# slp-rl/aero

Hardware: NVIDIA H100
Metric: audio-seconds/sec forward (higher is better)
Workload: dtype f16 tensor-core operands and activation storage (10-bit mantissa = tf32), fp32 accumulate / norm inputs / cell state

## Files before the change

### aero_b200/cabi.py

```python
from __future__ import annotations

import ctypes as C
import os

_HERE = os.path.dirname(os.path.abspath(__file__))
LIB_PATH = os.path.join(_HERE, "libaero_b200.so")

i32, i64, f32 = C.c_int32, C.c_int64, C.c_float
vp = C.c_void_p


class StftParams(C.Structure):
    _fields_ = [("n_fft", i32), ("hop", i32), ("win", i32), ("n_signals", i32), ("channels", i32),
                ("length", i32), ("frames", i32), ("bins_out", i32),
                ("z_stride_b", i64), ("z_stride_c", i64), ("z_stride_k", i64), ("z_stride_t", i64),
                ("flags", i32), ("reserved", i32)]


class IstftParams(C.Structure):
    _fields_ = [("n_fft", i32), ("hop", i32), ("win", i32), ("n_signals", i32), ("channels", i32),
                ("frames", i32), ("bins_in", i32), ("out_len", i32),
                ("z_stride_b", i64), ("z_stride_c", i64), ("z_stride_k", i64), ("z_stride_t", i64),
                ("flags", i32), ("reserved", i32)]

# ... 47 lines not shown
ACT_NONE, ACT_GELU, ACT_RELU, ACT_LEAKY, ACT_TANH = 0, 1, 2, 3, 4
TG_ROUND_TF32, TG_A_F16, TG_OUT_F16, TG_REVERSE = 1, 2, 4, 8
NA_NONE, NA_GELU, NA_GLU, NA_SNAKE, NA_GLU_SCALE_RES, NA_RELU, NA_LEAKY, NA_TANH = 0, 1, 2, 3, 4, 5, 6, 7
NA_NO_NORM = 16
STFT_ZERO_PAD, STFT_ADJ_SCALE, ISTFT_RAW = 1, 2, 1
GAN_NONE, GAN_LSGAN_REAL, GAN_LSGAN_FAKE, GAN_LSGAN_GEN, GAN_HINGE_REAL, GAN_HINGE_FAKE, GAN_HINGE_GEN = 0, 1, 2, 3, 4, 5, 6
GAN_FWD_BLOCKS = 128

SYMBOLS = {
    "aero_abi_version": (C.c_int, []),
    "aero_last_error": (C.c_char_p, []),
    "aero_device_arch": (C.c_int, []),
    "aero_launch_count": (C.c_uint64, []),
    "aero_stft_fwd": (C.c_int, [vp, vp, vp, vp, C.POINTER(StftParams), vp]),
    "aero_istft_fwd": (C.c_int, [vp, vp, vp, C.POINTER(IstftParams), vp]),
    "aero_tapgemm_fwd": (C.c_int, [vp] * 10 + [C.POINTER(TapGemmParams), vp]),
    "aero_tapgemm_tc_eligible": (C.c_int, [C.POINTER(TapGemmParams)]),
    "aero_sample_norm_fwd": (C.c_int, [vp, vp, vp, vp, i32, i64, i64, i32, vp]),
    "aero_norm_act_fwd": (C.c_int, [vp] * 8 + [C.POINTER(NormActParams), vp]),
    "aero_ftb_lin_out_fwd": (C.c_int, [vp] * 7 + [C.POINTER(FtbLinParams), vp]),
    "aero_ftb_lin_squeeze_fwd": (C.c_int, [vp, vp, vp, vp, i32, C.POINTER(FtbLinParams), vp]),
    "aero_freq_mix_small_fwd": (C.c_int, [vp, vp, vp, vp, i32, i32, i64, i32, vp]),
    "aero_lstm_rec_fwd": (C.c_int, [vp, vp, vp, vp, C.POINTER(LstmParams), vp]),
    "aero_local_attn_fwd": (C.c_int, [vp, vp, C.POINTER(AttnParams), vp]),
    "aero_lsd_fwd": (C.c_int, [vp, vp, vp, i32, i32, i32, i32, vp]),
    "aero_stft_loss_fwd": (C.c_int, [vp, vp, vp, i32, i32, i32, i32, vp]),
    "aero_stft_loss_bwd": (C.c_int, [vp, vp, vp, vp, i32, i32, i32, i32, f32, f32, vp]),
    "aero_tapgemm_wgrad": (C.c_int, [vp, vp, vp, vp, C.POINTER(TapGemmParams), i64, i64, i64, vp]),
    "aero_colsum": (C.c_int, [vp, vp, vp, vp, i32, i32, i64, i64, i64, i64, i32, i64, i64, vp]),
    "aero_add": (C.c_int, [vp, vp, i64, f32, vp]),
    "aero_add_f64": (C.c_int, [vp, vp, i64, vp]),
    "aero_gram": (C.c_int, [vp, vp, vp, vp, i32, i32, i64, i64, i64, i64, vp]),
    "aero_bcast_add": (C.c_int, [vp, vp, i32, i32, i32, i32, vp]),
    "aero_scale_rows": (C.c_int, [vp, vp, vp, i32, i64, i32, vp]),
    "aero_norm_act_train_fwd": (C.c_int, [vp] * 8 + [C.POINTER(NormActParams), vp]),
    "aero_norm_act_train_bwd": (C.c_int, [vp] * 13 + [i32, C.POINTER(NormActParams), vp]),
    "aero_adam_step": (C.c_int, [vp, i32, f32, f32, f32, f32, i32, f32, vp]),
    "aero_pack_kmajor_tf32": (C.c_int, [vp, vp, vp, i32, i32, i32, vp]),
    "aero_split_tf32": (C.c_int, [vp, vp, vp, i64, vp]),
    "aero_tapgemm_wgrad_tc_eligible": (C.c_int, [C.POINTER(TapGemmParams), vp, vp, vp]),
    "aero_gconv1d_fwd": (C.c_int, [vp, vp, vp, vp] + [i32] * 9 + [vp]),
    "aero_gconv1d_dgrad": (C.c_int, [vp, vp, vp] + [i32] * 9 + [vp]),
    "aero_gconv1d_wgrad": (C.c_int, [vp, vp, vp] + [i32] * 9 + [vp]),
    "aero_weight_norm_fwd": (C.c_int, [vp, vp, vp, i32, i32, vp]),
    "aero_weight_norm_bwd": (C.c_int, [vp, vp, vp, vp, vp, i32, i32, vp]),
    "aero_lstm_train_fwd": (C.c_int, [vp] * 7 + [C.POINTER(LstmParams), vp]),
# ... 54 lines not shown
```

### aero_b200/csrc/lstm_tc.cu

```cuda
#include <cuda_fp16.h>
#include <cstdlib>
#include "tc_common.cuh"

#ifdef AERO_TC_TRACE
__device__ long long g_lstm_trace[128 * 8];
#define LSTM_TRACE(slot, step) do { if (blockIdx.x == 0 && blockIdx.y == 0 && (step) < 128) g_lstm_trace[(step) * 8 + (slot)] = clock64(); } while (0)
extern "C" int aero_debug_lstm_trace(long long* host) {
    return cudaMemcpyFromSymbol(host, g_lstm_trace, sizeof(g_lstm_trace)) == cudaSuccess ? 0 : -1;
}
#else
#define LSTM_TRACE(slot, step) do { } while (0)
#endif

namespace aero {

constexpr int kNT = 16;
constexpr int kLdAcc = kNT + 4;

static int lstm_seq_knob() {
    static const int v = [] { const char* e = getenv("AERO_LSTM_SEQ"); return e ? atoi(e) : 0; }();
    return v;
}

struct LstmTcShared {
    uint64_t w_full;
    uint64_t acc_ready;
    uint64_t h_ready;
};

__device__ __forceinline__ float fast_ex2(float x) {
    float y;
    asm("ex2.approx.ftz.f32 %0, %1;" : "=f"(y) : "f"(x));
    return y;
}
__device__ __forceinline__ float fast_rcp(float x) {
    float y;
    asm("rcp.approx.ftz.f32 %0, %1;" : "=f"(y) : "f"(x));
    return y;
}

template <typename T> __device__ __forceinline__ T to_storage(float v);
template <> __device__ __forceinline__ float to_storage<float>(float v) { return v; }
template <> __device__ __forceinline__ __half to_storage<__half>(float v) { return __float2half_rn(v); }

template <int GPT, int NEW, int SEQ, int ROWB, int MINB, typename TO, typename TG>
__global__ void __launch_bounds__(128 + 32 * NEW, MINB)
lstm_tc_kernel(const __grid_constant__ CUtensorMap mapW, const TG* __restrict__ gin, const float* __restrict__ bias_pad,
               TO* __restrict__ hout, const aero_lstm_params p, const int nK) {
    constexpr int NM = 4 / GPT;
    constexpr int CPW = 32 / GPT;
    constexpr int kNS = 4 * SEQ / NEW;
    constexpr int kATile = 128 * ROWB, kBTile = kNT * ROWB, kKC = ROWB / 2;
    extern __shared__ uint8_t smem_raw[];
    uint8_t* smem = reinterpret_cast<uint8_t*>((reinterpret_cast<uintptr_t>(smem_raw) + 1023) & ~(uintptr_t)1023);
    uint8_t* sA = smem;
    uint8_t* sB = smem + NM * nK * kATile;
    float* sAcc = reinterpret_cast<float*>(sB + nK * kBTile);
    LstmTcShared* sh = reinterpret_cast<LstmTcShared*>(sAcc + NM * 128 * kLdAcc);

    const int warp = threadIdx.x >> 5, lane = threadIdx.x & 31;
    const int dir = blockIdx.y;
    const int seq0 = blockIdx.x * SEQ;
    const int n_seq = p.rows * p.n_win;
    const int H = p.H;
    const int ldg = 8 * H;

    if (threadIdx.x == 0) {
        mbar_init(&sh->w_full, 1);
        mbar_init(&sh->acc_ready, 128);
        mbar_init(&sh->h_ready, 32 * NEW);
        asm volatile("fence.mbarrier_init.release.cluster;" ::: "memory");
    }
    for (int i = threadIdx.x; i < nK * kBTile / 4; i += blockDim.x) reinterpret_cast<float*>(sB)[i] = 0.f;
    fence_proxy_async_smem();
    __syncthreads();

    if (warp < 4) {
        if (threadIdx.x == 0) {
            asm volatile("prefetch.tensormap [%0];" ::"l"(&mapW) : "memory");
            mbar_expect_tx(&sh->w_full, (uint32_t)(NM * nK * kATile));
            for (int m = 0; m < NM; ++m)
                for (int kc = 0; kc < nK; ++kc)
                    tma_load_2d(sA + (m * nK + kc) * kATile, &mapW, &sh->w_full, kc * kKC, (dir * NM + m) * 128);
        }
        constexpr int kMaxKC = (ROWB == 128) ? 2 : 4;
        uint64_t da[NM][kMaxKC], db[kMaxKC];
        const uint32_t a0 = smem_u32(sA), b0 = smem_u32(sB);
#pragma unroll
        for (int kc = 0; kc < kMaxKC; ++kc) {
            db[kc] = make_desc_kmajor<ROWB>(b0 + (uint32_t)(kc * kBTile));
#pragma unroll
            for (int m = 0; m < NM; ++m) da[m][kc] = make_desc_kmajor<ROWB>(a0 + (uint32_t)((m * nK + kc) * kATile));
        }
        float* const arow = sAcc + (warp * 16 + (lane >> 2)) * kLdAcc + 2 * (lane & 3);
        mbar_wait(&sh->w_full, 0);
        for (int s = 1; s < p.steps; ++s) {
            mbar_wait(&sh->h_ready, (uint32_t)((s - 1) & 1));
            LSTM_TRACE(0, s);
            float d[NM][2][8];
            wgmma_fence();
#pragma unroll
            for (int m = 0; m < NM; ++m) {
#pragma unroll
                for (int hf = 0; hf < 2; ++hf) {
#pragma unroll
                    for (int kc = 0; kc < kMaxKC; ++kc) {
                        if (kc < nK) {
#pragma unroll
                            for (int k = 0; k < ROWB / 32; ++k)
                                Wgmma<kNT, true, 0>::ss(d[m][hf], da[m][kc] + (uint64_t)(hf * ((64 * ROWB) >> 4) + 2 * k), db[kc] + 2 * k,
                                                        (kc == 0 && k == 0) ? 0u : 1u);
                        }
                    }
                }
            }
            wgmma_commit();
            wgmma_wait<0>();
#pragma unroll
            for (int m = 0; m < NM; ++m)
#pragma unroll
                for (int hf = 0; hf < 2; ++hf)
#pragma unroll
                    for (int j = 0; j < 2; ++j) {
                        float* r = arow + (m * 128 + hf * 64) * kLdAcc + 8 * j;
                        *reinterpret_cast<float2*>(r) = make_float2(d[m][hf][4 * j], d[m][hf][4 * j + 1]);
                        *reinterpret_cast<float2*>(r + 8 * kLdAcc) = make_float2(d[m][hf][4 * j + 2], d[m][hf][4 * j + 3]);
                    }
            mbar_arrive(&sh->acc_ready);
            LSTM_TRACE(1, s);
        }
    } else {
        const int ew = warp - 4;
        const int q = warp & 3;
        const int wp = ew >> 2;
        const int sub = lane / CPW;
        const int cell = q * CPW + (lane % CPW);
        const bool cell_ok = cell < H;
        const int r = q * 32 + lane;
        const int half = p.win_stride / 2;
        const int dpos = dir ? -1 : 1;
        const int pos0 = dir ? p.steps - 1 : 0;

        const int gcol = dir * 4 * H + sub * H + min(cell, H - 1);
        const int gtile = GPT * H;
        constexpr int kMS = kNS / GPT;
        int goff[kNS], g_lo[kNS], g_len[kNS];
        int ooff[kMS], w_lo[kMS], w_len[kMS];
        uint32_t baddr[kMS];
        const int jq = (cell & (kKC - 1)) >> 3;
        const uint32_t bbase = smem_u32(sB) + (uint32_t)((cell / kKC) * kBTile + ((cell & 7) << 1));
#pragma unroll
        for (int i = 0; i < kNS; ++i) {
            const int n = wp * kNS + i;
            const int sq = min(seq0 + n, n_seq - 1);
            const int row = sq / p.n_win, k = sq - row * p.n_win;
            const int f0 = k * p.win_stride;
            goff[i] = (p.in_windowed ? (sq * p.steps + pos0) : (row * p.T + f0 + pos0)) * ldg + gcol;
            const int in_hi = p.in_windowed ? p.steps : max(0, min(p.steps, p.T - f0));
            g_lo[i] = dir ? p.steps - in_hi : 0;
            g_len[i] = in_hi;
        }
#pragma unroll
        for (int ii = 0; ii < kMS; ++ii) {
            const int n = wp * kNS + ii * GPT + sub;
            const int sq = min(seq0 + n, n_seq - 1);
            const bool exists = seq0 + n < n_seq;
            const int row = sq / p.n_win, k = sq - row * p.n_win;
            const int f0 = k * p.win_stride;
            ooff[ii] = (p.out_windowed ? (sq * p.steps + pos0) : (row * p.T + f0 + pos0)) * 2 * H + dir * H + cell;
            int lo = 0, hi = p.steps;
            if (!p.out_windowed) {
                lo = (k == 0) ? 0 : half;
                hi = min((k == p.n_win - 1) ? p.steps : p.steps - half, p.T - f0);
            }
            if (!exists || !cell_ok) hi = lo;
            w_lo[ii] = dir ? p.steps - hi : lo;
            w_len[ii] = max(0, hi - lo);
            baddr[ii] = bbase + (uint32_t)((n >> 3) * (8 * ROWB) + (n & 7) * ROWB + ((jq ^ (ROWB == 128 ? (n & 7) : ((n >> 1) & 3))) << 4));
        }
        const float* bptr = bias_pad + gcol;
        const int gstep = dpos * ldg, ostep = dpos * 2 * H;

        float c_state[kMS];
#pragma unroll
        for (int i = 0; i < kMS; ++i) c_state[i] = 0.f;

        constexpr bool kRegPrefetch = (GPT == 1);
        TG gn[kRegPrefetch ? NM : 1][kRegPrefetch ? kNS : 1];
        const TG* const bptr_g = nullptr;
        (void)bptr_g;
        if (kRegPrefetch) {
#pragma unroll
            for (int i = 0; i < kNS; ++i) {
                const bool real = (unsigned)(0 - g_lo[i]) < (unsigned)g_len[i];
#pragma unroll
                for (int m = 0; m < NM; ++m) gn[kRegPrefetch ? m : 0][kRegPrefetch ? i : 0] = real ? gin[goff[i] + m * gtile] : to_storage<TG>(bptr[m * gtile]);
                goff[i] += gstep;
            }
        }
        for (int s = 0; s < p.steps; ++s) {
            float gi[NM][kNS];
            if (kRegPrefetch) {
#pragma unroll
                for (int i = 0; i < kNS; ++i) {
#pragma unroll
                    for (int m = 0; m < NM; ++m) gi[m][i] = ldf(&gn[kRegPrefetch ? m : 0][kRegPrefetch ? i : 0]);
                }
                if (s + 1 < p.steps) {
#pragma unroll
                    for (int i = 0; i < kNS; ++i) {
                        const bool real = (unsigned)(s + 1 - g_lo[i]) < (unsigned)g_len[i];
#pragma unroll
                        for (int m = 0; m < NM; ++m) gn[kRegPrefetch ? m : 0][kRegPrefetch ? i : 0] = real ? gin[goff[i] + m * gtile] : to_storage<TG>(bptr[m * gtile]);
                        goff[i] += gstep;
                    }
                }
            } else {
#pragma unroll
                for (int i = 0; i < kNS; ++i) {
                    const bool real = (unsigned)(s - g_lo[i]) < (unsigned)g_len[i];
#pragma unroll
                    for (int m = 0; m < NM; ++m) gi[m][i] = real ? ldf(gin + goff[i] + m * gtile) : bptr[m * gtile];
                    goff[i] += gstep;
                }
            }
            if (ew == 0 && lane == 0) LSTM_TRACE(2, s);
            if (s > 0) {
                mbar_wait(&sh->acc_ready, (uint32_t)((s - 1) & 1));
            }
            if (ew == 0 && lane == 0) LSTM_TRACE(3, s);
            float a[NM][kNS];
#pragma unroll
            for (int m = 0; m < NM; ++m) {
                uint32_t acc[kNS];
                if (s > 0) {
                    const uint32_t arow = smem_u32(sAcc + (m * 128 + r) * kLdAcc + wp * kNS);
#pragma unroll
                    for (int i = 0; i < kNS; i += 4) {
                        const float4 v = lds128(arow + 4u * i);
                        acc[i] = __float_as_uint(v.x); acc[i + 1] = __float_as_uint(v.y); acc[i + 2] = __float_as_uint(v.z); acc[i + 3] = __float_as_uint(v.w);
                    }
                } else {
#pragma unroll
                    for (int i = 0; i < kNS; ++i) acc[i] = 0u;
                }
                const int gate = m * GPT + sub;
                const float k_in = (gate == 2) ? -2.885390081777927f : -1.4426950408889634f;
                const float k_mul = (gate == 2) ? 2.0f : 1.0f, k_add = (gate == 2) ? -1.0f : 0.0f;
#pragma unroll
                for (int i = 0; i < kNS; ++i) {
                    const float x = __uint_as_float(acc[i]) + gi[m][i];
                    a[m][i] = fmaf(k_mul, fast_rcp(1.0f + fast_ex2(k_in * x)), k_add);
                }
            }
            if (ew == 0 && lane == 0) LSTM_TRACE(4, s);
#pragma unroll
            for (int ii = 0; ii < kMS; ++ii) {
                float ig, fg, gg, og;
                if (GPT == 1) {
                    ig = a[0][ii]; fg = a[1 % NM][ii]; gg = a[2 % NM][ii]; og = a[3 % NM][ii];
                } else {
                    const int e = (2 * ii) % kNS, o = (2 * ii + 1) % kNS;
                    const float own0 = sub ? a[0][o] : a[0][e], own1 = sub ? a[1 % NM][o] : a[1 % NM][e];
                    const float snd0 = sub ? a[0][e] : a[0][o], snd1 = sub ? a[1 % NM][e] : a[1 % NM][o];
                    const float p0 = __shfl_xor_sync(0xffffffffu, snd0, 16);
                    const float p1 = __shfl_xor_sync(0xffffffffu, snd1, 16);
                    if (sub == 0) { ig = own0; gg = own1; fg = p0; og = p1; }
                    else          { fg = own0; og = own1; ig = p0; gg = p1; }
                }
                const float c = fmaf(fg, c_state[ii], ig * gg);
                c_state[ii] = c;
                const float th = fmaf(2.0f, fast_rcp(1.0f + fast_ex2(-2.885390081777927f * c)), -1.0f);
                const float h = round_tf32_rna(og * th);
                if (cell_ok) {
                    const unsigned short hh = __half_as_ushort(__float2half_rn(h));
                    asm volatile("st.shared.u16 [%0], %1;" ::"r"(baddr[ii]), "h"(hh) : "memory");
                }
                if ((unsigned)(s - w_lo[ii]) < (unsigned)w_len[ii]) stf(hout + ooff[ii], h);
                ooff[ii] += ostep;
            }
            if (ew == 0 && lane == 0) LSTM_TRACE(5, s);
            if (s + 1 < p.steps) {
                fence_proxy_async_smem();
                mbar_arrive(&sh->h_ready);
            }
            if (ew == 0 && lane == 0) LSTM_TRACE(6, s);
        }
    }
}

template <int GPT, int NEW, int SEQ, int ROWB, int MINB, typename TO>
static void lstm_tc_go(dim3 grid, size_t smem, cudaStream_t st, const CUtensorMap& mW, const void* gin, const float* bias_pad, void* hout,
                       const aero_lstm_params& p, int nK) {
    if (p.flags & AERO_TG_A_F16) {
        cudaFuncSetAttribute(lstm_tc_kernel<GPT, NEW, SEQ, ROWB, MINB, TO, __half>, cudaFuncAttributeMaxDynamicSharedMemorySize, (int)smem);
        lstm_tc_kernel<GPT, NEW, SEQ, ROWB, MINB, TO, __half><<<grid, 128 + 32 * NEW, smem, st>>>(mW, static_cast<const __half*>(gin), bias_pad,
                                                                                              static_cast<TO*>(hout), p, nK);
    } else {
        cudaFuncSetAttribute(lstm_tc_kernel<GPT, NEW, SEQ, ROWB, MINB, TO, float>, cudaFuncAttributeMaxDynamicSharedMemorySize, (int)smem);
        lstm_tc_kernel<GPT, NEW, SEQ, ROWB, MINB, TO, float><<<grid, 128 + 32 * NEW, smem, st>>>(mW, static_cast<const float*>(gin), bias_pad,
                                                                                             static_cast<TO*>(hout), p, nK);
    }
}

int lstm_tc_launch(const void* gin, const float* bias_pad, const void* whh_r, void* hout, const aero_lstm_params& p,
                   cudaStream_t st) {
    const int H = p.H;
    if (H % 4 || H <= 32 || H > 128) {
        set_error("aero_lstm_rec_fwd(wgmma): hidden size %d unsupported (multiple of 4 in (32, 128])", H);
        return AERO_ERR_UNSUPPORTED;
    }
    static int num_sms = 0;
    if (num_sms == 0) {
        int dev = 0;
        cudaGetDevice(&dev);
        cudaDeviceGetAttribute(&num_sms, cudaDevAttrMultiProcessorCount, dev);
    }
    const int n_seq = p.rows * p.n_win;
    const int gpt = H <= 64 ? 2 : 1;
    const int nM = 4 / gpt;
    const int Kp = ((H + 63) / 64) * 64;
    const int knob = lstm_seq_knob();
    const bool small = knob ? knob == 8 : (int64_t)cdiv(n_seq, 8) * 2 <= (int64_t)num_sms * (gpt == 1 ? 1 : 2);
    const int rowb = (gpt == 1 && small) ? 64 : 128;
    const int kc_elems = rowb / 2;
    const int nK = (H + kc_elems - 1) / kc_elems;
    CUtensorMap mW;
    uint64_t dims[2] = {(uint64_t)Kp, (uint64_t)(2 * nM * 128)};
    uint64_t strides[1] = {(uint64_t)Kp * 2};
    uint32_t box[2] = {(uint32_t)kc_elems, 128};
    int rc = encode_map(&mW, whh_r, 2, dims, strides, box, rowb == 64 ? 2 : 0, 2);
    if (rc != AERO_OK) return rc;
    const size_t smem = (size_t)nM * nK * 128 * rowb + (size_t)nK * kNT * rowb + (size_t)nM * 128 * kLdAcc * 4 + sizeof(LstmTcShared) + 1024;
    if (smem > 227 * 1024) {
        set_error("aero_lstm_rec_fwd(wgmma): hidden size %d needs %zu bytes of shared memory", H, smem);
        return AERO_ERR_UNSUPPORTED;
    }
    const int64_t max_rows = (int64_t)n_seq * p.steps > (int64_t)p.rows * p.T ? (int64_t)n_seq * p.steps : (int64_t)p.rows * p.T;
    if ((max_rows + p.steps) * (8ll * H) >= (1ll << 31)) {
        set_error("aero_lstm_rec_fwd(wgmma): problem too large for 32-bit offsets (%lld rows)", (long long)max_rows);
        return AERO_ERR_UNSUPPORTED;
    }
    dim3 grid(cdiv(n_seq, small ? 8 : kNT), 2);
    const bool o16 = p.flags & AERO_TG_OUT_F16;
#define AERO_LSTM_GO(GPT, NEW, SEQ, ROWB, MINB)                                                              \
    do {                                                                                                      \
        if (o16) lstm_tc_go<GPT, NEW, SEQ, ROWB, MINB, __half>(grid, smem, st, mW, gin, bias_pad, hout, p, nK); \
        else lstm_tc_go<GPT, NEW, SEQ, ROWB, MINB, float>(grid, smem, st, mW, gin, bias_pad, hout, p, nK);      \
    } while (0)
    if (gpt == 1) {
        if (small) AERO_LSTM_GO(1, 8, 8, 64, 1);
        else AERO_LSTM_GO(1, 16, 16, 128, 1);
    } else {
        if (small) AERO_LSTM_GO(2, 8, 8, 128, 2);
        else AERO_LSTM_GO(2, 8, 16, 128, 2);
    }
#undef AERO_LSTM_GO
    return check_launch("aero_lstm_rec_fwd(wgmma)");
}

}
```

### aero_b200/csrc/wgmma.cuh

```cuda
#pragma once
#include <cstdint>

namespace aero {

__device__ __forceinline__ void wgmma_fence() { asm volatile("wgmma.fence.sync.aligned;" ::: "memory"); }
__device__ __forceinline__ void wgmma_commit() { asm volatile("wgmma.commit_group.sync.aligned;" ::: "memory"); }
template <int PENDING>
__device__ __forceinline__ void wgmma_wait() { asm volatile("wgmma.wait_group.sync.aligned %0;" ::"n"(PENDING) : "memory"); }

template <int ROWB>
__device__ __forceinline__ uint64_t make_desc_kmajor(uint32_t saddr) {
    return (uint64_t)((saddr >> 4) & 0x3FFF) | ((uint64_t)1 << 16) | ((uint64_t)((ROWB * 8) >> 4) << 32) |
           ((uint64_t)(ROWB == 128 ? 1 : 2) << 62);
}
__device__ __forceinline__ uint64_t make_desc_sw128(uint32_t saddr) { return make_desc_kmajor<128>(saddr); }

template <int N, bool F16, int TA> struct Wgmma;

template <int TA> struct Wgmma<16, true, TA> {
    static __device__ __forceinline__ void ss(float (&d)[8], uint64_t da, uint64_t db, uint32_t acc) {
        asm volatile("{\n\t.reg .pred p;\n\tsetp.ne.b32 p, %10, 0;\n\t"
                     "wgmma.mma_async.sync.aligned.m64n16k16.f32.f16.f16 {%0, %1, %2, %3, %4, %5, %6, %7}, %8, %9, p, 1, 1, %11, 0;\n\t}"
            : "+f"(d[0]), "+f"(d[1]), "+f"(d[2]), "+f"(d[3]), "+f"(d[4]), "+f"(d[5]), "+f"(d[6]), "+f"(d[7])
            : "l"(da), "l"(db), "r"(acc), "n"(TA));
    }
};
template <> struct Wgmma<16, false, 0> {
    static __device__ __forceinline__ void ss(float (&d)[8], uint64_t da, uint64_t db, uint32_t acc) {
        asm volatile("{\n\t.reg .pred p;\n\tsetp.ne.b32 p, %10, 0;\n\t"
                     "wgmma.mma_async.sync.aligned.m64n16k8.f32.tf32.tf32 {%0, %1, %2, %3, %4, %5, %6, %7}, %8, %9, p, 1, 1;\n\t}"
            : "+f"(d[0]), "+f"(d[1]), "+f"(d[2]), "+f"(d[3]), "+f"(d[4]), "+f"(d[5]), "+f"(d[6]), "+f"(d[7])
            : "l"(da), "l"(db), "r"(acc));
    }
    static __device__ __forceinline__ void rs(float (&d)[8], const uint32_t (&a)[4], uint64_t db, uint32_t acc) {
        asm volatile("{\n\t.reg .pred p;\n\tsetp.ne.b32 p, %13, 0;\n\t"
                     "wgmma.mma_async.sync.aligned.m64n16k8.f32.tf32.tf32 {%0, %1, %2, %3, %4, %5, %6, %7}, {%8, %9, %10, %11}, %12, p, 1, 1;\n\t}"
            : "+f"(d[0]), "+f"(d[1]), "+f"(d[2]), "+f"(d[3]), "+f"(d[4]), "+f"(d[5]), "+f"(d[6]), "+f"(d[7])
            : "r"(a[0]), "r"(a[1]), "r"(a[2]), "r"(a[3]), "l"(db), "r"(acc));
    }
};

template <int TA> struct Wgmma<32, true, TA> {
    static __device__ __forceinline__ void ss(float (&d)[16], uint64_t da, uint64_t db, uint32_t acc) {
        asm volatile("{\n\t.reg .pred p;\n\tsetp.ne.b32 p, %18, 0;\n\t"
                     "wgmma.mma_async.sync.aligned.m64n32k16.f32.f16.f16 {%0, %1, %2, %3, %4, %5, %6, %7, %8, %9, %10, %11, %12, %13, %14, %15}, %16, %17, p, 1, 1, %19, 0;\n\t}"
            : "+f"(d[0]), "+f"(d[1]), "+f"(d[2]), "+f"(d[3]), "+f"(d[4]), "+f"(d[5]), "+f"(d[6]), "+f"(d[7]),
              "+f"(d[8]), "+f"(d[9]), "+f"(d[10]), "+f"(d[11]), "+f"(d[12]), "+f"(d[13]), "+f"(d[14]), "+f"(d[15])
// ... 285 lines not shown
```

### include/aero_b200.h

```cpp
#ifndef AERO_B200_H
#define AERO_B200_H

#include <stddef.h>
#include <stdint.h>

#ifdef __cplusplus
extern "C" {
#endif

typedef void* aero_stream_t;

enum aero_status {
    AERO_OK = 0,
    AERO_ERR_INVALID = -1,
    AERO_ERR_UNSUPPORTED = -2,
    AERO_ERR_LAUNCH = -3,
    AERO_ERR_NO_DEVICE = -4
};

int aero_abi_version(void);
const char* aero_last_error(void);
int aero_device_arch(void);
uint64_t aero_launch_count(void);

// ... 75 lines not shown

typedef struct {
    int32_t B, F, T, N, J;
    int32_t flags;
    int64_t z_sb, z_sf, zm_sb, zm_sf;
} aero_ftb_lin_params;
int aero_ftb_lin_out_fwd(const float* z, const float* zm, const float* M, const float* s, const float* V, const float* d,
                         void* out, const aero_ftb_lin_params* p, aero_stream_t stream);
int aero_ftb_lin_squeeze_fwd(const float* z, const float* W1p, const float* b1p, void* R, int32_t r,
                             const aero_ftb_lin_params* p, aero_stream_t stream);

int aero_freq_mix_small_fwd(const void* x, const float* W, const float* gate, void* out, int32_t B, int32_t F, int64_t M,
                            int32_t flags, aero_stream_t stream);

typedef struct {
    int32_t rows, T, H;
    int32_t n_win, steps, win_stride;
    int32_t in_windowed, out_windowed;
    int32_t flags;
    int32_t precision;
} aero_lstm_params;
int aero_lstm_rec_fwd(const void* gin, const float* bias_pad, const void* whh, void* hout,
                      const aero_lstm_params* p, aero_stream_t stream);

typedef struct {
    int32_t rows, T, H, heads, ndecay, ld;
    int32_t flags;
} aero_attn_params;
int aero_local_attn_fwd(const float* qkvd, void* out, const aero_attn_params* p, aero_stream_t stream);

int aero_lsd_fwd(const float* z_ref, const float* z_est, double* out_sum, int32_t B, int32_t bins, int32_t frames,
                 int32_t n_fft, aero_stream_t stream);

int aero_stft_loss_fwd(const float* z_est, const float* z_ref, double* sums, int32_t B, int32_t bins, int32_t frames,
                       int32_t n_fft, aero_stream_t stream);

int aero_stft_loss_bwd(const float* z_est, const float* z_ref, const double* sums, float* g_est, int32_t B, int32_t bins,
                       int32_t frames, int32_t n_fft, float c_sc, float c_mag, aero_stream_t stream);


int aero_tapgemm_wgrad(const float* a1, const float* a2, const float* dy, float* dw, const aero_tapgemm_params* p,
                       int64_t dw_sn, int64_t dw_sk, int64_t dw_ss, aero_stream_t stream);

int aero_colsum(const float* x, const float* z, void* out1, void* out2, int32_t out_double, int32_t N, int64_t n_inner,
                int64_t inner_stride, int64_t n_outer, int64_t outer_stride, int32_t n_seg, int64_t seg_stride_x,
                int64_t seg_stride_out, aero_stream_t stream);
// ... 111 lines not shown
```

Before: 3506.

## Restructure LSTM recurrence kernel with register-resident weights and double-buffered sequence groups

Rewrites the wgmma LSTM recurrent kernel so the recurrent weights live in registers (RS-form wgmma) instead of being TMA-loaded into shared memory. Each CTA handles two sequence groups ping-ponged through separate mbarriers, so the matmul of one group can overlap the cell update of the other. Cell threads now process pairs of cells with vectorized loads and stores. Tile width and sequences per CTA are chosen adaptively from SM count, and a shape-query entry point is exported. The supported hidden size drops from 128 to 96, and register pressure from holding the weights is a risk.

```diff
diff --git a/aero_b200/cabi.py b/aero_b200/cabi.py
--- a/aero_b200/cabi.py
+++ b/aero_b200/cabi.py
@@ -93,6 +93,7 @@
     "aero_ftb_lin_squeeze_fwd": (C.c_int, [vp, vp, vp, vp, i32, C.POINTER(FtbLinParams), vp]),
     "aero_freq_mix_small_fwd": (C.c_int, [vp, vp, vp, vp, i32, i32, i64, i32, vp]),
     "aero_lstm_rec_fwd": (C.c_int, [vp, vp, vp, vp, C.POINTER(LstmParams), vp]),
+    "aero_lstm_tc_shape": (C.c_int, [i32, i32, i32, C.POINTER(i32)]),
     "aero_local_attn_fwd": (C.c_int, [vp, vp, C.POINTER(AttnParams), vp]),
     "aero_lsd_fwd": (C.c_int, [vp, vp, vp, i32, i32, i32, i32, vp]),
     "aero_stft_loss_fwd": (C.c_int, [vp, vp, vp, i32, i32, i32, i32, vp]),
diff --git a/aero_b200/csrc/lstm_tc.cu b/aero_b200/csrc/lstm_tc.cu
--- a/aero_b200/csrc/lstm_tc.cu
+++ b/aero_b200/csrc/lstm_tc.cu
@@ -1,5 +1,5 @@
 #include <cuda_fp16.h>
-#include <cstdlib>
+#include <algorithm>
 #include "tc_common.cuh"
 
 #ifdef AERO_TC_TRACE
@@ -14,18 +14,16 @@
 
 namespace aero {
 
-constexpr int kNT = 16;
-constexpr int kLdAcc = kNT + 4;
-
-static int lstm_seq_knob() {
-    static const int v = [] { const char* e = getenv("AERO_LSTM_SEQ"); return e ? atoi(e) : 0; }();
-    return v;
-}
+constexpr int kCellThreads = 128;
+constexpr int kItems = 3;
+
+struct LstmTcShape {
+    int S, nt, ctas_per_dir, tps;
+};
 
 struct LstmTcShared {
-    uint64_t w_full;
-    uint64_t acc_ready;
-    uint64_t h_ready;
+    uint64_t acc_ready[2];
+    uint64_t h_ready[2];
 };
 
 __device__ __forceinline__ float fast_ex2(float x) {
@@ -39,275 +37,262 @@
     return y;
 }
 
-template <typename T> __device__ __forceinline__ T to_storage(float v);
-template <> __device__ __forceinline__ float to_storage<float>(float v) { return v; }
-template <> __device__ __forceinline__ __half to_storage<__half>(float v) { return __float2half_rn(v); }
-
-template <int GPT, int NEW, int SEQ, int ROWB, int MINB, typename TO, typename TG>
-__global__ void __launch_bounds__(128 + 32 * NEW, MINB)
-lstm_tc_kernel(const __grid_constant__ CUtensorMap mapW, const TG* __restrict__ gin, const float* __restrict__ bias_pad,
-               TO* __restrict__ hout, const aero_lstm_params p, const int nK) {
-    constexpr int NM = 4 / GPT;
-    constexpr int CPW = 32 / GPT;
-    constexpr int kNS = 4 * SEQ / NEW;
-    constexpr int kATile = 128 * ROWB, kBTile = kNT * ROWB, kKC = ROWB / 2;
+__device__ __forceinline__ float2 ld2f(const float* p) { return *reinterpret_cast<const float2*>(p); }
+__device__ __forceinline__ float2 to_f2(float2 v) { return v; }
+__device__ __forceinline__ float2 to_f2(__half2 v) { return __half22float2(v); }
+template <typename TG> struct Pair;
+template <> struct Pair<float> { using T = float2; };
+template <> struct Pair<__half> { using T = __half2; };
+__device__ __forceinline__ void st2(float* p, float a, float b) { *reinterpret_cast<float2*>(p) = make_float2(a, b); }
+__device__ __forceinline__ void st2(__half* p, float a, float b) { *reinterpret_cast<uint32_t*>(p) = pack_half2_sat(a, b); }
+
+template <int KS> struct LstmTcCfg {
+    static constexpr int kWG = KS > 4 ? 2 : 1;
+    static constexpr int kTW = (KS + kWG - 1) / kWG;
+    static constexpr int kLdr = 64 * kWG * kTW + 4;
+    static constexpr int kThreads = 128 * kWG + 2 * kCellThreads;
+};
+
+template <int KS, int NT, typename TO, typename TG>
+__global__ void __launch_bounds__(LstmTcCfg<KS>::kThreads, 1)
+lstm_tc_kernel(const __half* __restrict__ whh, const TG* __restrict__ gin, const float* __restrict__ bias_pad,
+               TO* __restrict__ hout, const aero_lstm_params p, const int S, const int tps) {
+    using Cfg = LstmTcCfg<KS>;
+    constexpr int kTW = Cfg::kTW, kLdr = Cfg::kLdr, NWG = Cfg::kWG;
+    constexpr int nK = (KS + 3) / 4;
+    constexpr int kBTile = NT * 128;
+    using TG2 = typename Pair<TG>::T;
     extern __shared__ uint8_t smem_raw[];
     uint8_t* smem = reinterpret_cast<uint8_t*>((reinterpret_cast<uintptr_t>(smem_raw) + 1023) & ~(uintptr_t)1023);
-    uint8_t* sA = smem;
-    uint8_t* sB = smem + NM * nK * kATile;
-    float* sAcc = reinterpret_cast<float*>(sB + nK * kBTile);
-    LstmTcShared* sh = reinterpret_cast<LstmTcShared*>(sAcc + NM * 128 * kLdAcc);
+    const int H = p.H;
+    uint8_t* sB = smem;
+    float* sAcc = reinterpret_cast<float*>(sB + 2 * nK * kBTile);
+    LstmTcShared* sh = reinterpret_cast<LstmTcShared*>(sAcc + 2 * NT * kLdr);
 
     const int warp = threadIdx.x >> 5, lane = threadIdx.x & 31;
     const int dir = blockIdx.y;
-    const int seq0 = blockIdx.x * SEQ;
     const int n_seq = p.rows * p.n_win;
-    const int H = p.H;
-    const int ldg = 8 * H;
+    const int seq0 = blockIdx.x * 2 * S;
+    const int live0 = min(S, n_seq - seq0), live1 = max(0, min(S, n_seq - seq0 - S));
 
     if (threadIdx.x == 0) {
-        mbar_init(&sh->w_full, 1);
-        mbar_init(&sh->acc_ready, 128);
-        mbar_init(&sh->h_ready, 32 * NEW);
+        for (int g = 0; g < 2; ++g) {
+            mbar_init(&sh->acc_ready[g], 128 * NWG);
+            mbar_init(&sh->h_ready[g], max(1, (g ? live1 : live0) * tps));
+        }
         asm volatile("fence.mbarrier_init.release.cluster;" ::: "memory");
     }
-    for (int i = threadIdx.x; i < nK * kBTile / 4; i += blockDim.x) reinterpret_cast<float*>(sB)[i] = 0.f;
+    for (int i = threadIdx.x; i < 2 * nK * kBTile / 4; i += blockDim.x) reinterpret_cast<float*>(sB)[i] = 0.f;
     fence_proxy_async_smem();
     __syncthreads();
 
-    if (warp < 4) {
-        if (threadIdx.x == 0) {
-            asm volatile("prefetch.tensormap [%0];" ::"l"(&mapW) : "memory");
-            mbar_expect_tx(&sh->w_full, (uint32_t)(NM * nK * kATile));
-            for (int m = 0; m < NM; ++m)
-                for (int kc = 0; kc < nK; ++kc)
-                    tma_load_2d(sA + (m * nK + kc) * kATile, &mapW, &sh->w_full, kc * kKC, (dir * NM + m) * 128);
-        }
-        constexpr int kMaxKC = (ROWB == 128) ? 2 : 4;
-        uint64_t da[NM][kMaxKC], db[kMaxKC];
-        const uint32_t a0 = smem_u32(sA), b0 = smem_u32(sB);
-#pragma unroll
-        for (int kc = 0; kc < kMaxKC; ++kc) {
-            db[kc] = make_desc_kmajor<ROWB>(b0 + (uint32_t)(kc * kBTile));
-#pragma unroll
-            for (int m = 0; m < NM; ++m) da[m][kc] = make_desc_kmajor<ROWB>(a0 + (uint32_t)((m * nK + kc) * kATile));
-        }
-        float* const arow = sAcc + (warp * 16 + (lane >> 2)) * kLdAcc + 2 * (lane & 3);
-        mbar_wait(&sh->w_full, 0);
+    if (warp < 4 * NWG) {
+        const int wg = warp >> 2, wl = warp & 3;
+        const int kp = 64 * nK;
+        const int nM = H > 64 ? 4 : 2;
+        uint32_t a[kTW][KS][4];
+#pragma unroll
+        for (int lt = 0; lt < kTW; ++lt)
+#pragma unroll
+            for (int k = 0; k < KS; ++k)
+#pragma unroll
+                for (int r = 0; r < 4; ++r) {
+                    const int R = (wg * kTW + lt) * 64 + wl * 16 + (lane >> 2) + 8 * (r & 1);
+                    const int col = 16 * k + 2 * (lane & 3) + 8 * (r >> 1);
+                    uint32_t v = 0u;
+                    if (R < 4 * H && col < H) {
+                        const int gate = R / H, cell = R - gate * H;
+                        const int src = H > 64 ? gate * 128 + cell
+                                               : (gate >> 1) * 128 + (cell >> 4) * 32 + (gate & 1) * 16 + (cell & 15);
+                        v = __ldg(reinterpret_cast<const uint32_t*>(whh + (size_t)(dir * nM * 128 + src) * kp + col));
+                    }
+                    a[lt][k][r] = v;
+                }
+        const uint64_t db0 = make_desc_kmajor<128>(smem_u32(sB));
+        const int ng = live1 > 0 ? 2 : 1;
+        float* const arow = sAcc + 2 * (lane & 3) * kLdr + wg * kTW * 64 + wl * 16 + (lane >> 2);
         for (int s = 1; s < p.steps; ++s) {
-            mbar_wait(&sh->h_ready, (uint32_t)((s - 1) & 1));
-            LSTM_TRACE(0, s);
-            float d[NM][2][8];
-            wgmma_fence();
-#pragma unroll
-            for (int m = 0; m < NM; ++m) {
-#pragma unroll
-                for (int hf = 0; hf < 2; ++hf) {
-#pragma unroll
-                    for (int kc = 0; kc < kMaxKC; ++kc) {
-                        if (kc < nK) {
-#pragma unroll
-                            for (int k = 0; k < ROWB / 32; ++k)
-                                Wgmma<kNT, true, 0>::ss(d[m][hf], da[m][kc] + (uint64_t)(hf * ((64 * ROWB) >> 4) + 2 * k), db[kc] + 2 * k,
-                                                        (kc == 0 && k == 0) ? 0u : 1u);
-                        }
-                    }
-                }
-            }
-            wgmma_commit();
-            wgmma_wait<0>();
-#pragma unroll
-            for (int m = 0; m < NM; ++m)
-#pragma unroll
-                for (int hf = 0; hf < 2; ++hf)
-#pragma unroll
-                    for (int j = 0; j < 2; ++j) {
-                        float* r = arow + (m * 128 + hf * 64) * kLdAcc + 8 * j;
-                        *reinterpret_cast<float2*>(r) = make_float2(d[m][hf][4 * j], d[m][hf][4 * j + 1]);
-                        *reinterpret_cast<float2*>(r + 8 * kLdAcc) = make_float2(d[m][hf][4 * j + 2], d[m][hf][4 * j + 3]);
-                    }
-            mbar_arrive(&sh->acc_ready);
-            LSTM_TRACE(1, s);
+            for (int g = 0; g < ng; ++g) {
+                mbar_wait(&sh->h_ready[g], (uint32_t)((s - 1) & 1));
+                if (g == 0) LSTM_TRACE(0, s);
+                const uint64_t db = db0 + (uint64_t)(g * ((nK * kBTile) >> 4));
+                float d[kTW][NT / 2];
+                wgmma_fence();
+#pragma unroll
+                for (int lt = 0; lt < kTW; ++lt)
+#pragma unroll
+                    for (int k = 0; k < KS; ++k)
+                        Wgmma<NT, true, 0>::rs(d[lt], a[lt][k], db + (uint64_t)((k >> 2) * (kBTile >> 4) + 2 * (k & 3)), k == 0 ? 0u : 1u);
+                wgmma_commit();
+                wgmma_wait<0>();
+                float* const acc = arow + g * NT * kLdr;
+#pragma unroll
+                for (int lt = 0; lt < kTW; ++lt)
+#pragma unroll
+                    for (int j = 0; j < NT / 8; ++j)
+#pragma unroll
+                        for (int e = 0; e < 4; ++e)
+                            acc[(8 * j + (e & 1)) * kLdr + lt * 64 + 8 * (e >> 1)] = d[lt][4 * j + e];
+                mbar_arrive(&sh->acc_ready[g]);
+                if (g == 0) LSTM_TRACE(1, s);
+            }
         }
     } else {
-        const int ew = warp - 4;
-        const int q = warp & 3;
-        const int wp = ew >> 2;
-        const int sub = lane / CPW;
-        const int cell = q * CPW + (lane % CPW);
-        const bool cell_ok = cell < H;
-        const int r = q * 32 + lane;
+        const int g = (warp - 4 * NWG) >> 2;
+        const int t = threadIdx.x - 128 * NWG - g * kCellThreads;
+        const int n = t / tps, pp = t - n * tps;
+        if (n >= (g ? live1 : live0)) return;
+        const int hp = H >> 1;
         const int half = p.win_stride / 2;
         const int dpos = dir ? -1 : 1;
         const int pos0 = dir ? p.steps - 1 : 0;
-
-        const int gcol = dir * 4 * H + sub * H + min(cell, H - 1);
-        const int gtile = GPT * H;
-        constexpr int kMS = kNS / GPT;
-        int goff[kNS], g_lo[kNS], g_len[kNS];
-        int ooff[kMS], w_lo[kMS], w_len[kMS];
-        uint32_t baddr[kMS];
-        const int jq = (cell & (kKC - 1)) >> 3;
-        const uint32_t bbase = smem_u32(sB) + (uint32_t)((cell / kKC) * kBTile + ((cell & 7) << 1));
-#pragma unroll
-        for (int i = 0; i < kNS; ++i) {
-            const int n = wp * kNS + i;
-            const int sq = min(seq0 + n, n_seq - 1);
-            const int row = sq / p.n_win, k = sq - row * p.n_win;
-            const int f0 = k * p.win_stride;
-            goff[i] = (p.in_windowed ? (sq * p.steps + pos0) : (row * p.T + f0 + pos0)) * ldg + gcol;
-            const int in_hi = p.in_windowed ? p.steps : max(0, min(p.steps, p.T - f0));
-            g_lo[i] = dir ? p.steps - in_hi : 0;
-            g_len[i] = in_hi;
-        }
-#pragma unroll
-        for (int ii = 0; ii < kMS; ++ii) {
-            const int n = wp * kNS + ii * GPT + sub;
-            const int sq = min(seq0 + n, n_seq - 1);
-            const bool exists = seq0 + n < n_seq;
-            const int row = sq / p.n_win, k = sq - row * p.n_win;
-            const int f0 = k * p.win_stride;
-            ooff[ii] = (p.out_windowed ? (sq * p.steps + pos0) : (row * p.T + f0 + pos0)) * 2 * H + dir * H + cell;
-            int lo = 0, hi = p.steps;
-            if (!p.out_windowed) {
-                lo = (k == 0) ? 0 : half;
-                hi = min((k == p.n_win - 1) ? p.steps : p.steps - half, p.T - f0);
-            }
-            if (!exists || !cell_ok) hi = lo;
-            w_lo[ii] = dir ? p.steps - hi : lo;
-            w_len[ii] = max(0, hi - lo);
-            baddr[ii] = bbase + (uint32_t)((n >> 3) * (8 * ROWB) + (n & 7) * ROWB + ((jq ^ (ROWB == 128 ? (n & 7) : ((n >> 1) & 3))) << 4));
-        }
-        const float* bptr = bias_pad + gcol;
+        const int ldg = 8 * H;
+
+        const int sq = seq0 + g * S + n;
+        const int row = sq / p.n_win, k = sq - row * p.n_win;
+        const int f0 = k * p.win_stride;
+        const int cell0 = 2 * pp, cstep = 2 * tps;
+        const int gcol = dir * 4 * H + cell0;
+        int goff = (p.in_windowed ? (sq * p.steps + pos0) : (row * p.T + f0 + pos0)) * ldg + gcol;
+        const int in_hi = p.in_windowed ? p.steps : max(0, min(p.steps, p.T - f0));
+        const int g_lo = dir ? p.steps - in_hi : 0, g_len = in_hi;
+        int ooff = (p.out_windowed ? (sq * p.steps + pos0) : (row * p.T + f0 + pos0)) * 2 * H + dir * H + cell0;
+        int lo = 0, hi = p.steps;
+        if (!p.out_windowed) {
+            lo = (k == 0) ? 0 : half;
+            hi = min((k == p.n_win - 1) ? p.steps : p.steps - half, p.T - f0);
+        }
+        const int w_lo = dir ? p.steps - hi : lo, w_len = max(0, hi - lo);
+        const float* const accn = sAcc + (g * NT + n) * kLdr + cell0;
+        bool ok[kItems];
+        uint32_t baddr[kItems];
+#pragma unroll
+        for (int j = 0; j < kItems; ++j) {
+            ok[j] = pp + tps * j < hp;
+            const int cell = cell0 + cstep * j;
+            baddr[j] = smem_u32(sB) + (uint32_t)((g * nK + (cell >> 6)) * kBTile + (n >> 3) * 1024 + (n & 7) * 128 +
+                                                 ((((cell & 63) >> 3) ^ (n & 7)) << 4) + ((cell & 7) << 1));
+        }
         const int gstep = dpos * ldg, ostep = dpos * 2 * H;
 
-        float c_state[kMS];
-#pragma unroll
-        for (int i = 0; i < kMS; ++i) c_state[i] = 0.f;
-
-        constexpr bool kRegPrefetch = (GPT == 1);
-        TG gn[kRegPrefetch ? NM : 1][kRegPrefetch ? kNS : 1];
-        const TG* const bptr_g = nullptr;
-        (void)bptr_g;
-        if (kRegPrefetch) {
-#pragma unroll
-            for (int i = 0; i < kNS; ++i) {
-                const bool real = (unsigned)(0 - g_lo[i]) < (unsigned)g_len[i];
-#pragma unroll
-                for (int m = 0; m < NM; ++m) gn[kRegPrefetch ? m : 0][kRegPrefetch ? i : 0] = real ? gin[goff[i] + m * gtile] : to_storage<TG>(bptr[m * gtile]);
-                goff[i] += gstep;
-            }
-        }
+        float c_state[kItems][2];
+        TG2 gn[kItems][4];
+#pragma unroll
+        for (int j = 0; j < kItems; ++j) {
+            c_state[j][0] = c_state[j][1] = 0.f;
+            if (ok[j] && (unsigned)(0 - g_lo) < (unsigned)g_len) {
+#pragma unroll
+                for (int q = 0; q < 4; ++q) gn[j][q] = *reinterpret_cast<const TG2*>(gin + goff + cstep * j + q * H);
+            }
+        }
+        goff += gstep;
         for (int s = 0; s < p.steps; ++s) {
-            float gi[NM][kNS];
-            if (kRegPrefetch) {
-#pragma unroll
-                for (int i = 0; i < kNS; ++i) {
-#pragma unroll
-                    for (int m = 0; m < NM; ++m) gi[m][i] = ldf(&gn[kRegPrefetch ? m : 0][kRegPrefetch ? i : 0]);
-                }
-                if (s + 1 < p.steps) {
-#pragma unroll
-                    for (int i = 0; i < kNS; ++i) {
-                        const bool real = (unsigned)(s + 1 - g_lo[i]) < (unsigned)g_len[i];
-#pragma unroll
-                        for (int m = 0; m < NM; ++m) gn[kRegPrefetch ? m : 0][kRegPrefetch ? i : 0] = real ? gin[goff[i] + m * gtile] : to_storage<TG>(bptr[m * gtile]);
-                        goff[i] += gstep;
-                    }
-                }
-            } else {
-#pragma unroll
-                for (int i = 0; i < kNS; ++i) {
-                    const bool real = (unsigned)(s - g_lo[i]) < (unsigned)g_len[i];
-#pragma unroll
-                    for (int m = 0; m < NM; ++m) gi[m][i] = real ? ldf(gin + goff[i] + m * gtile) : bptr[m * gtile];
-                    goff[i] += gstep;
-                }
-            }
-            if (ew == 0 && lane == 0) LSTM_TRACE(2, s);
-            if (s > 0) {
-                mbar_wait(&sh->acc_ready, (uint32_t)((s - 1) & 1));
-            }
-            if (ew == 0 && lane == 0) LSTM_TRACE(3, s);
-            float a[NM][kNS];
-#pragma unroll
-            for (int m = 0; m < NM; ++m) {
-                uint32_t acc[kNS];
-                if (s > 0) {
-                    const uint32_t arow = smem_u32(sAcc + (m * 128 + r) * kLdAcc + wp * kNS);
-#pragma unroll
-                    for (int i = 0; i < kNS; i += 4) {
-                        const float4 v = lds128(arow + 4u * i);
-                        acc[i] = __float_as_uint(v.x); acc[i + 1] = __float_as_uint(v.y); acc[i + 2] = __float_as_uint(v.z); acc[i + 3] = __float_as_uint(v.w);
-                    }
-                } else {
-#pragma unroll
-                    for (int i = 0; i < kNS; ++i) acc[i] = 0u;
-                }
-                const int gate = m * GPT + sub;
-                const float k_in = (gate == 2) ? -2.885390081777927f : -1.4426950408889634f;
-                const float k_mul = (gate == 2) ? 2.0f : 1.0f, k_add = (gate == 2) ? -1.0f : 0.0f;
-#pragma unroll
-                for (int i = 0; i < kNS; ++i) {
-                    const float x = __uint_as_float(acc[i]) + gi[m][i];
-                    a[m][i] = fmaf(k_mul, fast_rcp(1.0f + fast_ex2(k_in * x)), k_add);
-                }
-            }
-            if (ew == 0 && lane == 0) LSTM_TRACE(4, s);
-#pragma unroll
-            for (int ii = 0; ii < kMS; ++ii) {
-                float ig, fg, gg, og;
-                if (GPT == 1) {
-                    ig = a[0][ii]; fg = a[1 % NM][ii]; gg = a[2 % NM][ii]; og = a[3 % NM][ii];
-                } else {
-                    const int e = (2 * ii) % kNS, o = (2 * ii + 1) % kNS;
-                    const float own0 = sub ? a[0][o] : a[0][e], own1 = sub ? a[1 % NM][o] : a[1 % NM][e];
-                    const float snd0 = sub ? a[0][e] : a[0][o], snd1 = sub ? a[1 % NM][e] : a[1 % NM][o];
-                    const float p0 = __shfl_xor_sync(0xffffffffu, snd0, 16);
-                    const float p1 = __shfl_xor_sync(0xffffffffu, snd1, 16);
-                    if (sub == 0) { ig = own0; gg = own1; fg = p0; og = p1; }
-                    else          { fg = own0; og = own1; ig = p0; gg = p1; }
-                }
-                const float c = fmaf(fg, c_state[ii], ig * gg);
-                c_state[ii] = c;
-                const float th = fmaf(2.0f, fast_rcp(1.0f + fast_ex2(-2.885390081777927f * c)), -1.0f);
-                const float h = round_tf32_rna(og * th);
-                if (cell_ok) {
-                    const unsigned short hh = __half_as_ushort(__float2half_rn(h));
-                    asm volatile("st.shared.u16 [%0], %1;" ::"r"(baddr[ii]), "h"(hh) : "memory");
-                }
-                if ((unsigned)(s - w_lo[ii]) < (unsigned)w_len[ii]) stf(hout + ooff[ii], h);
-                ooff[ii] += ostep;
-            }
-            if (ew == 0 && lane == 0) LSTM_TRACE(5, s);
+            float2 gi[kItems][4];
+            const bool real = (unsigned)(s - g_lo) < (unsigned)g_len;
+            const bool real_next = s + 1 < p.steps && (unsigned)(s + 1 - g_lo) < (unsigned)g_len;
+            const bool real_next2 = s + 2 < p.steps && (unsigned)(s + 2 - g_lo) < (unsigned)g_len;
+#pragma unroll
+            for (int j = 0; j < kItems; ++j) {
+                if (!ok[j]) continue;
+#pragma unroll
+                for (int q = 0; q < 4; ++q) gi[j][q] = real ? to_f2(gn[j][q]) : ld2f(bias_pad + gcol + cstep * j + q * H);
+                if (real_next) {
+#pragma unroll
+                    for (int q = 0; q < 4; ++q) gn[j][q] = *reinterpret_cast<const TG2*>(gin + goff + cstep * j + q * H);
+                }
+                if (real_next2) {
+#pragma unroll
+                    for (int q = 0; q < 4; ++q)
+                        asm volatile("prefetch.global.L2 [%0];" ::"l"(gin + goff + gstep + cstep * j + q * H));
+                }
+            }
+            goff += gstep;
+            if (g == 0 && t == 0) LSTM_TRACE(2, s);
+            if (s > 0) mbar_wait(&sh->acc_ready[g], (uint32_t)((s - 1) & 1));
+            if (g == 0 && t == 0) LSTM_TRACE(3, s);
+            const bool store = (unsigned)(s - w_lo) < (unsigned)w_len;
+#pragma unroll
+            for (int j = 0; j < kItems; ++j) {
+                if (!ok[j]) continue;
+                float act[4][2];
+#pragma unroll
+                for (int q = 0; q < 4; ++q) {
+                    const float2 acc = s > 0 ? *reinterpret_cast<const float2*>(accn + cstep * j + q * H) : make_float2(0.f, 0.f);
+                    const float k_in = (q == 2) ? -2.885390081777927f : -1.4426950408889634f;
+                    const float k_mul = (q == 2) ? 2.0f : 1.0f, k_add = (q == 2) ? -1.0f : 0.0f;
+                    act[q][0] = fmaf(k_mul, fast_rcp(1.0f + fast_ex2(k_in * (acc.x + gi[j][q].x))), k_add);
+                    act[q][1] = fmaf(k_mul, fast_rcp(1.0f + fast_ex2(k_in * (acc.y + gi[j][q].y))), k_add);
+                }
+                float h[2];
+#pragma unroll
+                for (int e = 0; e < 2; ++e) {
+                    const float c = fmaf(act[1][e], c_state[j][e], act[0][e] * act[2][e]);
+                    c_state[j][e] = c;
+                    const float th = fmaf(2.0f, fast_rcp(1.0f + fast_ex2(-2.885390081777927f * c)), -1.0f);
+                    h[e] = round_tf32_rna(act[3][e] * th);
+                }
+                const __half2 hh = __floats2half2_rn(h[0], h[1]);
+                asm volatile("st.shared.b32 [%0], %1;" ::"r"(baddr[j]), "r"(*reinterpret_cast<const uint32_t*>(&hh)) : "memory");
+                if (store) st2(hout + ooff + cstep * j, h[0], h[1]);
+            }
+            ooff += ostep;
+            if (g == 0 && t == 0) LSTM_TRACE(5, s);
             if (s + 1 < p.steps) {
                 fence_proxy_async_smem();
-                mbar_arrive(&sh->h_ready);
-            }
-            if (ew == 0 && lane == 0) LSTM_TRACE(6, s);
-        }
-    }
-}
-
-template <int GPT, int NEW, int SEQ, int ROWB, int MINB, typename TO>
-static void lstm_tc_go(dim3 grid, size_t smem, cudaStream_t st, const CUtensorMap& mW, const void* gin, const float* bias_pad, void* hout,
-                       const aero_lstm_params& p, int nK) {
+                mbar_arrive(&sh->h_ready[g]);
+            }
+            if (g == 0 && t == 0) LSTM_TRACE(6, s);
+        }
+    }
+}
+
+template <int KS, int NT, typename TO>
+static void lstm_tc_go(dim3 grid, size_t smem, cudaStream_t st, const void* whh, const void* gin, const float* bias_pad, void* hout,
+                       const aero_lstm_params& p, const LstmTcShape& sp) {
+    const __half* w = static_cast<const __half*>(whh);
+    constexpr int kThreads = LstmTcCfg<KS>::kThreads;
     if (p.flags & AERO_TG_A_F16) {
-        cudaFuncSetAttribute(lstm_tc_kernel<GPT, NEW, SEQ, ROWB, MINB, TO, __half>, cudaFuncAttributeMaxDynamicSharedMemorySize, (int)smem);
-        lstm_tc_kernel<GPT, NEW, SEQ, ROWB, MINB, TO, __half><<<grid, 128 + 32 * NEW, smem, st>>>(mW, static_cast<const __half*>(gin), bias_pad,
-                                                                                              static_cast<TO*>(hout), p, nK);
+        cudaFuncSetAttribute(lstm_tc_kernel<KS, NT, TO, __half>, cudaFuncAttributeMaxDynamicSharedMemorySize, (int)smem);
+        lstm_tc_kernel<KS, NT, TO, __half><<<grid, kThreads, smem, st>>>(w, static_cast<const __half*>(gin), bias_pad,
+                                                                         static_cast<TO*>(hout), p, sp.S, sp.tps);
     } else {
-        cudaFuncSetAttribute(lstm_tc_kernel<GPT, NEW, SEQ, ROWB, MINB, TO, float>, cudaFuncAttributeMaxDynamicSharedMemorySize, (int)smem);
-        lstm_tc_kernel<GPT, NEW, SEQ, ROWB, MINB, TO, float><<<grid, 128 + 32 * NEW, smem, st>>>(mW, static_cast<const float*>(gin), bias_pad,
-                                                                                             static_cast<TO*>(hout), p, nK);
-    }
+        cudaFuncSetAttribute(lstm_tc_kernel<KS, NT, TO, float>, cudaFuncAttributeMaxDynamicSharedMemorySize, (int)smem);
+        lstm_tc_kernel<KS, NT, TO, float><<<grid, kThreads, smem, st>>>(w, static_cast<const float*>(gin), bias_pad,
+                                                                        static_cast<TO*>(hout), p, sp.S, sp.tps);
+    }
+}
+
+template <int KS>
+static void lstm_tc_dispatch(dim3 grid, cudaStream_t st, const void* whh, const void* gin, const float* bias_pad, void* hout,
+                             const aero_lstm_params& p, const LstmTcShape& sp) {
+    const size_t smem = 1024 + 2 * (size_t)((KS + 3) / 4) * sp.nt * 128 + 2 * (size_t)sp.nt * LstmTcCfg<KS>::kLdr * 4 + sizeof(LstmTcShared);
+    const bool o16 = p.flags & AERO_TG_OUT_F16;
+    constexpr int kWide = KS == 6 ? 8 : 16;
+    if (sp.nt == 8) {
+        if (o16) lstm_tc_go<KS, 8, __half>(grid, smem, st, whh, gin, bias_pad, hout, p, sp);
+        else lstm_tc_go<KS, 8, float>(grid, smem, st, whh, gin, bias_pad, hout, p, sp);
+    } else {
+        if (o16) lstm_tc_go<KS, kWide, __half>(grid, smem, st, whh, gin, bias_pad, hout, p, sp);
+        else lstm_tc_go<KS, kWide, float>(grid, smem, st, whh, gin, bias_pad, hout, p, sp);
+    }
+}
+
+LstmTcShape lstm_tc_shape(int n_seq, int H, int num_sms) {
+    LstmTcShape r;
+    r.tps = cdiv(H / 2, kItems);
+    const int per_dir = std::max(1, num_sms / 2);
+    const int cap = std::min((H + 15) / 16 == 6 ? 8 : 16, kCellThreads / r.tps);
+    r.S = std::max(1, std::min(cap, cdiv(n_seq, 2 * per_dir)));
+    r.nt = r.S <= 8 ? 8 : 16;
+    r.ctas_per_dir = cdiv(n_seq, 2 * r.S);
+    return r;
 }
 
 int lstm_tc_launch(const void* gin, const float* bias_pad, const void* whh_r, void* hout, const aero_lstm_params& p,
                    cudaStream_t st) {
     const int H = p.H;
-    if (H % 4 || H <= 32 || H > 128) {
-        set_error("aero_lstm_rec_fwd(wgmma): hidden size %d unsupported (multiple of 4 in (32, 128])", H);
+    if (H % 4 || H <= 32 || H > 96) {
+        set_error("aero_lstm_rec_fwd(wgmma): hidden size %d unsupported (multiple of 4 in (32, 96])", H);
         return AERO_ERR_UNSUPPORTED;
     }
     static int num_sms = 0;
@@ -317,46 +302,30 @@
         cudaDeviceGetAttribute(&num_sms, cudaDevAttrMultiProcessorCount, dev);
     }
     const int n_seq = p.rows * p.n_win;
-    const int gpt = H <= 64 ? 2 : 1;
-    const int nM = 4 / gpt;
-    const int Kp = ((H + 63) / 64) * 64;
-    const int knob = lstm_seq_knob();
-    const bool small = knob ? knob == 8 : (int64_t)cdiv(n_seq, 8) * 2 <= (int64_t)num_sms * (gpt == 1 ? 1 : 2);
-    const int rowb = (gpt == 1 && small) ? 64 : 128;
-    const int kc_elems = rowb / 2;
-    const int nK = (H + kc_elems - 1) / kc_elems;
-    CUtensorMap mW;
-    uint64_t dims[2] = {(uint64_t)Kp, (uint64_t)(2 * nM * 128)};
-    uint64_t strides[1] = {(uint64_t)Kp * 2};
-    uint32_t box[2] = {(uint32_t)kc_elems, 128};
-    int rc = encode_map(&mW, whh_r, 2, dims, strides, box, rowb == 64 ? 2 : 0, 2);
-    if (rc != AERO_OK) return rc;
-    const size_t smem = (size_t)nM * nK * 128 * rowb + (size_t)nK * kNT * rowb + (size_t)nM * 128 * kLdAcc * 4 + sizeof(LstmTcShared) + 1024;
-    if (smem > 227 * 1024) {
-        set_error("aero_lstm_rec_fwd(wgmma): hidden size %d needs %zu bytes of shared memory", H, smem);
-        return AERO_ERR_UNSUPPORTED;
-    }
+    const LstmTcShape sp = lstm_tc_shape(n_seq, H, num_sms);
     const int64_t max_rows = (int64_t)n_seq * p.steps > (int64_t)p.rows * p.T ? (int64_t)n_seq * p.steps : (int64_t)p.rows * p.T;
     if ((max_rows + p.steps) * (8ll * H) >= (1ll << 31)) {
         set_error("aero_lstm_rec_fwd(wgmma): problem too large for 32-bit offsets (%lld rows)", (long long)max_rows);
         return AERO_ERR_UNSUPPORTED;
     }
-    dim3 grid(cdiv(n_seq, small ? 8 : kNT), 2);
-    const bool o16 = p.flags & AERO_TG_OUT_F16;
-#define AERO_LSTM_GO(GPT, NEW, SEQ, ROWB, MINB)                                                              \
-    do {                                                                                                      \
-        if (o16) lstm_tc_go<GPT, NEW, SEQ, ROWB, MINB, __half>(grid, smem, st, mW, gin, bias_pad, hout, p, nK); \
-        else lstm_tc_go<GPT, NEW, SEQ, ROWB, MINB, float>(grid, smem, st, mW, gin, bias_pad, hout, p, nK);      \
-    } while (0)
-    if (gpt == 1) {
-        if (small) AERO_LSTM_GO(1, 8, 8, 64, 1);
-        else AERO_LSTM_GO(1, 16, 16, 128, 1);
-    } else {
-        if (small) AERO_LSTM_GO(2, 8, 8, 128, 2);
-        else AERO_LSTM_GO(2, 8, 16, 128, 2);
-    }
-#undef AERO_LSTM_GO
+    const dim3 grid(sp.ctas_per_dir, 2);
+    switch ((H + 15) / 16) {
+        case 3: lstm_tc_dispatch<3>(grid, st, whh_r, gin, bias_pad, hout, p, sp); break;
+        case 4: lstm_tc_dispatch<4>(grid, st, whh_r, gin, bias_pad, hout, p, sp); break;
+        case 5: lstm_tc_dispatch<5>(grid, st, whh_r, gin, bias_pad, hout, p, sp); break;
+        default: lstm_tc_dispatch<6>(grid, st, whh_r, gin, bias_pad, hout, p, sp); break;
+    }
     return check_launch("aero_lstm_rec_fwd(wgmma)");
 }
 
 }
+
+extern "C" int aero_lstm_tc_shape(int32_t n_seq, int32_t H, int32_t num_sms, int32_t* out) {
+    if (!out || n_seq < 1 || H % 4 || H <= 32 || H > 96 || num_sms < 1) return AERO_ERR_INVALID;
+    const aero::LstmTcShape r = aero::lstm_tc_shape(n_seq, H, num_sms);
+    out[0] = r.S;
+    out[1] = r.nt;
+    out[2] = r.ctas_per_dir;
+    out[3] = r.tps;
+    return AERO_OK;
+}
diff --git a/aero_b200/csrc/wgmma.cuh b/aero_b200/csrc/wgmma.cuh
--- a/aero_b200/csrc/wgmma.cuh
+++ b/aero_b200/csrc/wgmma.cuh
@@ -17,12 +17,26 @@
 
 template <int N, bool F16, int TA> struct Wgmma;
 
+template <int TA> struct Wgmma<8, true, TA> {
+    static __device__ __forceinline__ void rs(float (&d)[4], const uint32_t (&a)[4], uint64_t db, uint32_t acc) {
+        asm volatile("{\n\t.reg .pred p;\n\tsetp.ne.b32 p, %9, 0;\n\t"
+                     "wgmma.mma_async.sync.aligned.m64n8k16.f32.f16.f16 {%0, %1, %2, %3}, {%4, %5, %6, %7}, %8, p, 1, 1, 0;\n\t}"
+            : "+f"(d[0]), "+f"(d[1]), "+f"(d[2]), "+f"(d[3])
+            : "r"(a[0]), "r"(a[1]), "r"(a[2]), "r"(a[3]), "l"(db), "r"(acc));
+    }
+};
 template <int TA> struct Wgmma<16, true, TA> {
     static __device__ __forceinline__ void ss(float (&d)[8], uint64_t da, uint64_t db, uint32_t acc) {
         asm volatile("{\n\t.reg .pred p;\n\tsetp.ne.b32 p, %10, 0;\n\t"
                      "wgmma.mma_async.sync.aligned.m64n16k16.f32.f16.f16 {%0, %1, %2, %3, %4, %5, %6, %7}, %8, %9, p, 1, 1, %11, 0;\n\t}"
             : "+f"(d[0]), "+f"(d[1]), "+f"(d[2]), "+f"(d[3]), "+f"(d[4]), "+f"(d[5]), "+f"(d[6]), "+f"(d[7])
             : "l"(da), "l"(db), "r"(acc), "n"(TA));
+    }
+    static __device__ __forceinline__ void rs(float (&d)[8], const uint32_t (&a)[4], uint64_t db, uint32_t acc) {
+        asm volatile("{\n\t.reg .pred p;\n\tsetp.ne.b32 p, %13, 0;\n\t"
+                     "wgmma.mma_async.sync.aligned.m64n16k16.f32.f16.f16 {%0, %1, %2, %3, %4, %5, %6, %7}, {%8, %9, %10, %11}, %12, p, 1, 1, 0;\n\t}"
+            : "+f"(d[0]), "+f"(d[1]), "+f"(d[2]), "+f"(d[3]), "+f"(d[4]), "+f"(d[5]), "+f"(d[6]), "+f"(d[7])
+            : "r"(a[0]), "r"(a[1]), "r"(a[2]), "r"(a[3]), "l"(db), "r"(acc));
     }
 };
 template <> struct Wgmma<16, false, 0> {
diff --git a/include/aero_b200.h b/include/aero_b200.h
--- a/include/aero_b200.h
+++ b/include/aero_b200.h
@@ -121,6 +121,7 @@
 } aero_lstm_params;
 int aero_lstm_rec_fwd(const void* gin, const float* bias_pad, const void* whh, void* hout,
                       const aero_lstm_params* p, aero_stream_t stream);
+int aero_lstm_tc_shape(int32_t n_seq, int32_t H, int32_t num_sms, int32_t* out);
 
 typedef struct {
     int32_t rows, T, H, heads, ndecay, ld;
```

Result: faster. 3724 (median of 6 runs) (+6.2%).
